# haowenz/FEM

Hardware: AMD Instinct MI355X
Metric: mapped Mreads/s (100 bp, e=3) at 1/2/4/8 MI355X + achieved HBM GB/s vs roofline (higher is better)
Workload: dtype u32/u64 integer + 32-bit Myers bit-vectors

## Files before the change

### fem_amd/csrc/fem_hip.hip

```cpp
#include "../../include/fem_hip.h"

#include <hip/hip_runtime.h>
#include <rccl/rccl.h>
#include <sched.h>
#if defined(__x86_64__)
#include <immintrin.h>
#endif

#include <algorithm>
#include <cctype>
#include <cstdio>
#include <cstdlib>
#include <cstring>
#include <condition_variable>
#include <functional>
#include <memory>
#include <atomic>
#include <chrono>
#include <mutex>
#include <string>
#include <thread>
#include <utility>
#include <vector>

// ... 199 lines not shown
  int n_cu = 256;
  std::string err;
  Buf<uint32_t> d_lookup;
  uint64_t n_lookup = 0;
  Buf<uint64_t> d_occ;
  uint64_t n_occ = 0;
  int32_t k = 0, step = 0;
  uint64_t fast_occ_key = ~0ull;
  int fast_occ_blocks = 0;
  Buf<uint32_t> d_summary;
  Buf<uint32_t> d_occ32, d_goff, d_blkseq;
  uint32_t list_shift = 0;
  bool no_strided = false;
  bool select_chars = false;
  bool verify_chars = false;
  Buf<uint32_t> d_freq11;
  uint32_t n_banks = 1, bank_first[5] = {0, 0, 0, 0, 0};
  Buf<uint32_t> d_bank_lo;
  uint64_t bank_limit = 0;
  uint32_t bank_seqs = 0;
  int select_occ_blocks = 0, join_occ_blocks = 0;
  uint64_t select_occ_key = ~0ull, join_occ_key = ~0ull;
  Buf<uint8_t> d_planes;
  Buf<uint8_t> d_ref_raw;
  uint64_t ref_bytes = 0;
  Buf<uint64_t> d_seq_off;
  Buf<uint32_t> d_seq_len;
  uint32_t n_seq = 0;
  std::vector<uint64_t> seq_off;
  std::vector<uint32_t> seq_len;
  Slot slot[kSlots];
// ... 167 lines not shown
    return at;
  };
  l.sf = take(2u * 64u * 4u);
  l.X = take(64u * 4u);
  l.A = take(3u * (femk::dense_flag_cap((int)R) + 1u) * 4u);
  l.B = take(2u * femk::kReadBlock * 8u);
  l.F = take(femk::join_bitmap_words((int)R, padded) * 4u);
  if (banked) l.gq = take(2u * 64u * 8u);
  l.wave_bytes = o;
  l.picked = 0;
  return l;
}

typedef void (*SeedKernel)(femk::SeedParams);
template <size_t... I>
SeedKernel select_kernel_of(int R, bool banked, bool packed, std::index_sequence<I...>) {
  static const SeedKernel k[2][2][femk::kMaxR] = {
      {{femk::seed_select_kernel<(int)I + 1, false, false>...}, {femk::seed_select_kernel<(int)I + 1, true, false>...}},
      {{femk::seed_select_kernel<(int)I + 1, false, true>...}, {femk::seed_select_kernel<(int)I + 1, true, true>...}}};
  return k[packed][banked][std::min(std::max(R, 1), femk::kMaxR) - 1];
}
template <size_t... I>
SeedKernel fast_kernel_of(int R, bool hash, std::index_sequence<I...>) {
  static const SeedKernel k[2][femk::kMaxR] = {{femk::seed_fast_kernel<(int)I + 1, false>...}, {femk::seed_fast_kernel<(int)I + 1, true>...}};
  return k[hash][std::min(std::max(R, 1), femk::kMaxR) - 1];
}
SeedKernel select_kernel(int R, bool banked, bool packed) { return select_kernel_of(R, banked, packed, std::make_index_sequence<femk::kMaxR>{}); }
SeedKernel fast_kernel(int R, bool hash) { return fast_kernel_of(R, hash, std::make_index_sequence<femk::kMaxR>{}); }
SeedKernel join_kernel(int R, int which) {
  static const SeedKernel k[3][femk::kMaxR] = {
      {femk::seed_join_kernel_r1, femk::seed_join_kernel_r2, femk::seed_join_kernel_r3, femk::seed_join_kernel_r4, femk::seed_join_kernel_r5,
       femk::seed_join_kernel_r6, femk::seed_join_kernel_r7, femk::seed_join_kernel_r8, femk::seed_join_kernel_r9, femk::seed_join_kernel_r10},
      {femk::seed_join_banked_kernel_r1, femk::seed_join_banked_kernel_r2, femk::seed_join_banked_kernel_r3, femk::seed_join_banked_kernel_r4,
       femk::seed_join_banked_kernel_r5, femk::seed_join_banked_kernel_r6, femk::seed_join_banked_kernel_r7, femk::seed_join_banked_kernel_r8,
       femk::seed_join_banked_kernel_r9, femk::seed_join_banked_kernel_r10},
      {femk::seed_join_kernel_padded_r1, femk::seed_join_kernel_padded_r2, femk::seed_join_kernel_padded_r3, femk::seed_join_kernel_padded_r4,
       femk::seed_join_kernel_padded_r5, femk::seed_join_kernel_padded_r6, femk::seed_join_kernel_padded_r7, femk::seed_join_kernel_padded_r8,
       femk::seed_join_kernel_padded_r9, femk::seed_join_kernel_padded_r10}};
  return k[which][std::min(std::max(R, 1), femk::kMaxR) - 1];
}

int blocks_per_cu(const void *kernel, int block, uint32_t lds) {
  int nb = 0;
  return hipOccupancyMaxActiveBlocksPerMultiprocessor(&nb, kernel, block, lds) == hipSuccess ? nb : 0;
}
uint32_t kernel_regs(int R, bool join, int which = 0, bool packed = false) {
  static std::atomic<uint32_t> cache[3][3][femk::kMaxR + 1] = {};
  std::atomic<uint32_t> &slot = cache[which][join ? 1 : packed ? 2 : 0][std::min(std::max(R, 1), femk::kMaxR)];
  uint32_t c = slot.load(std::memory_order_relaxed);
  if (c) return c;
  hipFuncAttributes a{};
  const void *f = join ? (const void *)join_kernel(R, which) : (const void *)select_kernel(R, which == 1, packed);
  c = hipFuncGetAttributes(&a, f) == hipSuccess && a.numRegs > 0 ? (uint32_t)a.numRegs : 128u;
  slot.store(c, std::memory_order_relaxed);
  return c;
}
void launch_select(int R, bool banked, dim3 grid, dim3 block, uint32_t lds, hipStream_t st, const femk::SeedParams &sp) {
  hipLaunchKernelGGL(select_kernel(R, banked, sp.packed != nullptr), grid, block, lds, st, sp);
}
void launch_join(int R, int which, dim3 grid, dim3 block, uint32_t lds, hipStream_t st, const femk::SeedParams &sp) {
  hipLaunchKernelGGL(join_kernel(R, which), grid, block, lds, st, sp);
}
void launch_fast(int R, bool hash, dim3 grid, dim3 block, uint32_t lds, hipStream_t st, const femk::SeedParams &sp) {
  hipLaunchKernelGGL(fast_kernel(R, hash), grid, block, lds, st, sp);
}

struct Span {
  fem_dev *h;
  Slot &s;
  hipStream_t st;
  TimedLaunch t;
  bool on;
  Span(fem_dev *h_, Slot &s_, int id, hipStream_t st_) : h(h_), s(s_), st(st_), t{id, nullptr, nullptr, false}, on(h_->timing && h_->timeline) {
// ... 153 lines not shown
}

int ensure_chars(fem_dev *h, Slot &s);

int launch_batch(fem_dev *h, Slot &s) {
  const fem_params &p = s.params;
  uint32_t *d_ctr = (uint32_t *)s.d_ctl.get();
  unsigned long long *d_arena_ctr = (unsigned long long *)(s.d_ctl + 4 * sizeof(uint32_t));
  unsigned long long *d_stats = (unsigned long long *)(s.d_ctl + 4 * sizeof(uint32_t) + 2 * sizeof(uint64_t));
  int parts = 1;
  uint32_t part_begin[kMaxParts + 1] = {0, 0, 0, 0, 0};
  const bool copied_in_parts = s.parts > 1;
  {
    const int R_ = p.e + 1 + p.a;
    const bool dense_overlap = !h->force_generic && p.k == femk::kK && p.step == femk::kStep && R_ >= 1 && R_ <= femk::kMaxR && h->d_occ32 &&
                               h->d_freq11 && !h->no_overlap;
    if (dense_overlap && !h->no_parts && s.n_reads >= 2 * kPartMinReads && (copied_in_parts || device_idle(h))) {
      parts = copied_in_parts ? s.parts : (int)std::min<uint64_t>((uint64_t)h->max_parts, s.n_reads / kPartMinReads);
      for (int q = 0; q <= parts; ++q)
        part_begin[q] = copied_in_parts ? s.part_begin[q] : q == parts ? (uint32_t)s.n_reads : (uint32_t)((s.n_reads * q / parts) & ~63ull);
    }
    s.parts = 1;
  }
  if (parts > 1) {
    if (h->have_select_done) HIP_TRY(h, hipStreamWaitEvent(h->side_stream, h->ev_select_done, 0));
    HIP_TRY(h, hipMemsetAsync(s.d_ctl, 0, kCtlAlloc, h->side_stream));
  } else {
    HIP_TRY(h, hipMemsetAsync(s.d_ctl, 0, kCtlAlloc, s.stream));
  }

  const int R_all = p.e + 1 + p.a;
  const bool dense_kernels = !h->force_generic && p.k == femk::kK && p.step == femk::kStep && R_all >= 1 && R_all <= femk::kMaxR && h->d_occ32 && h->d_freq11;
  if (s.n_reads && (!dense_kernels || h->verify_chars)) {
    int rc = ensure_chars(h, s);
    if (rc) return rc;
  }
  femk::SeedParams sp{};
  s.select_packed = false;
  if (s.sent_packed && !h->select_chars && dense_kernels) {
    sp.packed = s.packed(), sp.exc_bits = s.d_exc_bits, sp.bpr = s.packed_bpr, sp.len = s.max_len;
    s.select_packed = s.n_reads != 0;
  }
  sp.bases = s.bases();
  sp.read_off = s.d_off;
  sp.n_reads = (uint32_t)s.n_reads;
  sp.read_begin = 0;
  sp.lookup = h->d_lookup;
// ... 18 lines not shown
  const bool use_fast = !h->force_generic && p.k == femk::kK && p.step == femk::kStep && R >= 1 && R <= femk::kMaxR;

  auto shape = [&](const femk::SeedLayout &lay, uint32_t *wpb_out, uint32_t *lds_out, uint32_t *grid_out) {
    uint32_t wpb = std::min<uint32_t>(4u, std::max<uint32_t>(1u, (64u * 1024u) / lay.wave_bytes));
    uint32_t lds_bytes = wpb * lay.wave_bytes;
    uint32_t waves_per_cu = std::min<uint32_t>(32u, (160u * 1024u / lds_bytes) * wpb);
    uint64_t blocks_wanted = (s.n_reads + wpb - 1) / wpb;
    uint64_t blocks_resident = (uint64_t)h->n_cu * std::max<uint32_t>(1u, waves_per_cu / wpb);
    *wpb_out = wpb, *lds_out = lds_bytes;
    *grid_out = (uint32_t)std::max<uint64_t>(1, std::min<uint64_t>(blocks_wanted, blocks_resident * 4));
  };
  if (sp.lay.wave_bytes > 64u * 1024u) return fail(h, FEM_ERR_UNSUPPORTED, "read too long for the device path");

  if (s.n_reads) {
    int rc;
    const bool split_dense = use_fast && h->d_occ32 && h->d_freq11;
    const bool overlap = split_dense && !h->no_overlap;
    if (!overlap && h->have_kernels_done) HIP_TRY(h, hipStreamWaitEvent(s.stream, h->ev_kernels_done, 0));
    femk::VerifyParams vp{};
    vp.bases = s.bases(), vp.read_off = s.d_off;
    vp.planes = h->d_planes, vp.seq_off = h->d_seq_off;
    vp.cand = s.d_cand, vp.cand_meta = s.d_meta;
    vp.ctr = d_ctr, vp.cand_cap = s.cand_cap, vp.e = p.e;
    vp.ed = s.d_ed, vp.end = s.d_end;
    vp.n_map = s.d_nmap, vp.stats = d_stats;
    HIP_TRY(h, hipMemsetAsync(s.d_nmap, 0, (size_t)s.n_reads * sizeof(uint32_t), s.stream));
    const bool verify_packed = s.sent_packed && !h->verify_chars;
    if (verify_packed) vp.packed = s.packed(), vp.exc_bits = s.d_exc_bits, vp.bpr = s.packed_bpr, vp.len = s.max_len;
    void (*const verify)(femk::VerifyParams) = verify_packed ? femk::verify_kernel_packed : femk::verify_kernel;
    int &v_per_cu = verify_packed ? h->verify_packed_blocks_per_cu : h->verify_blocks_per_cu;
    if (v_per_cu == 0) {
      const int nb = blocks_per_cu((const void *)verify, 256, 0);
      v_per_cu = nb > 0 ? nb : 4;
    }
    const uint32_t vgrid = (uint32_t)h->n_cu * (uint32_t)v_per_cu;
    if (split_dense) {
      const uint32_t max_len = std::max<uint32_t>(s.max_len, (uint32_t)p.k);
      const bool banked = h->n_banks > 1;
      const size_t want_sel = (size_t)s.n_reads * 6u * (size_t)R * h->n_banks;
      HIP_TRY(h, s.d_sel.ensure(want_sel));
      HIP_TRY(h, s.d_sel_hdr.ensure((size_t)s.n_reads));
      femk::SeedParams fp = sp;
      fp.occ32 = h->d_occ32, fp.list_shift = h->list_shift, fp.goff = h->d_goff, fp.blkseq = h->d_blkseq;
      fp.freq11 = h->d_freq11, fp.sel = s.d_sel, fp.sel_hdr = s.d_sel_hdr;
      fp.n_banks = h->n_banks, fp.bank_lo = h->d_bank_lo, fp.n_buckets = (uint32_t)(h->n_lookup - 1);
      fp.blk_stride = (femk::kDenseRemap >> femk::kDenseBlkShift) + 1u;
      for (uint32_t b = 0; b <= femk::kDenseMaxBanks; ++b) fp.bank_first[b] = h->bank_first[b];
      uint32_t select_lds = 0, select_threads = 256;
      fp.lay = make_layout_select(p, max_len, fp.packed != nullptr);
      if (fp.lay.wave_bytes > 64u * 1024u) return fail(h, FEM_ERR_UNSUPPORTED, "read too long for the device path");
      const femk::SeedLayout lay_select = fp.lay;
      femk::SeedLayout lay_join = make_layout_join(p, banked, !banked && h->list_shift != 0);
      const uint32_t wpb_s = std::min<uint32_t>(4u, std::max<uint32_t>(1u, (64u * 1024u) / lay_select.wave_bytes));
      const uint32_t wpb_j = std::min<uint32_t>(4u, std::max<uint32_t>(1u, (60u * 1024u) / lay_join.wave_bytes));
      lay_join.picked = wpb_j * lay_join.wave_bytes;
      const uint32_t lds_j = wpb_j * lay_join.wave_bytes + 64u * 8u;
      const int which = banked ? 1 : h->list_shift ? 2 : 0;
      uint64_t per_cu_s, per_cu_j;
      {
        const uint32_t lds_bytes = wpb_s * lay_select.wave_bytes;
        const uint64_t key = ((uint64_t)(fp.packed != nullptr) << 49) | ((uint64_t)banked << 48) | ((uint64_t)R << 40) | lds_bytes;
        if (h->select_occ_key != key)
          h->select_occ_key = key, h->select_occ_blocks = blocks_per_cu((const void *)select_kernel(R, banked, fp.packed != nullptr), (int)(64u * wpb_s), lds_bytes);
        per_cu_s = h->select_occ_blocks > 0 ? (uint64_t)h->select_occ_blocks : std::max<uint64_t>(1, 160u * 1024u / lds_bytes);
        if (overlap) per_cu_s = 1;
        select_lds = lds_bytes, select_threads = 64u * wpb_s;
      }
      {
        const uint64_t key = ((uint64_t)which << 48) | ((uint64_t)R << 40) | lds_j;
        if (h->join_occ_key != key) h->join_occ_key = key, h->join_occ_blocks = blocks_per_cu((const void *)join_kernel(R, which), (int)(64u * wpb_j), lds_j);
        per_cu_j = h->join_occ_blocks > 0 ? (uint64_t)h->join_occ_blocks : std::max<uint64_t>(1, 160u * 1024u / lds_j);
        if (overlap) {
          const uint32_t vj = (kernel_regs(R, true, which) + 7u) & ~7u, vs = (kernel_regs(R, false, banked ? 1 : 0, fp.packed != nullptr) + 7u) & ~7u;
          const uint32_t wj = 64u * wpb_j / 256u ? 64u * wpb_j / 256u : 1u, ws = select_threads / 256u ? select_threads / 256u : 1u;
          const uint32_t lj = (lds_j + 511u) & ~511u, ls = (select_lds + 511u) & ~511u;
          while (per_cu_j > 1 && (per_cu_j * wj * vj + ws * vs > 512u || per_cu_j * lj + ls > 160u * 1024u || per_cu_j * wj + ws > 8u)) --per_cu_j;
        }
      }
      if (parts > 1 && !copied_in_parts) {
        HIP_TRY(h, hipEventRecord(s.ev_zeroed, s.stream));
        HIP_TRY(h, hipStreamWaitEvent(h->side_stream, s.ev_zeroed, 0));
      }
      for (int q = 0; q < parts; ++q) {
        const uint32_t r_lo = parts > 1 ? part_begin[q] : 0u, r_hi = parts > 1 ? part_begin[q + 1] : (uint32_t)s.n_reads;
        const uint64_t blocks_of_reads = ((uint64_t)(r_hi - r_lo) + femk::kReadBlock - 1) / femk::kReadBlock;
        fp.read_begin = r_lo, fp.n_reads = r_hi;
        hipStream_t st_sel = parts > 1 ? h->side_stream : s.stream;
        {
          fp.lay = lay_select;
          if (parts > 1) {
            if (copied_in_parts) HIP_TRY(h, hipStreamWaitEvent(st_sel, s.ev_part[q], 0));
          } else if (overlap && h->have_select_done) {
            HIP_TRY(h, hipStreamWaitEvent(s.stream, h->ev_select_done, 0));
          }
          const uint32_t grid = (uint32_t)std::max<uint64_t>(1, std::min<uint64_t>((blocks_of_reads + wpb_s - 1) / wpb_s, (uint64_t)h->n_cu * per_cu_s));
          fp.work_cursor = (uint32_t *)(s.d_ctl + kCtlWorkCursor + (size_t)q * kCtlPartStride);
          rc = timed_launch(h, s, 8, st_sel, q == 0, [&] { launch_select(R, banked, dim3(grid), dim3(64u * wpb_s), select_lds, st_sel, fp); });
          if (rc) return rc;
          if (parts > 1) {
            HIP_TRY(h, hipEventRecord(s.ev_sel[q], st_sel));
            HIP_TRY(h, hipStreamWaitEvent(s.stream, s.ev_sel[q], 0));
          }
          if (overlap && q + 1 == parts) {
            HIP_TRY(h, hipEventRecord(h->ev_select_done, st_sel));
            h->have_select_done = true;
          }
          if (overlap && q == 0 && h->have_kernels_done) HIP_TRY(h, hipStreamWaitEvent(s.stream, h->ev_kernels_done, 0));
        }
        {
          fp.lay = lay_join;
          const uint32_t grid = (uint32_t)std::max<uint64_t>(1, std::min<uint64_t>((blocks_of_reads + wpb_j - 1) / wpb_j, (uint64_t)h->n_cu * per_cu_j));
          fp.work_cursor = (uint32_t *)(s.d_ctl + kCtlWorkCursor2 + (size_t)q * kCtlPartStride);
// ... 75 lines not shown
  h->d_summary.release();
  const uint64_t n_buckets = h->n_lookup - 1;
  if (h->n_occ >= n_buckets || h->n_occ >= 0x80000000ull || (n_buckets >> 3) >= (1ull << 22)) return FEM_OK;
  const uint64_t words = n_buckets / femk::kSummaryBuckets + 2;
  HIP_TRY(h, h->d_summary.ensure(words));
  HIP_TRY(h, hipMemset(h->d_summary, 0, words * sizeof(uint32_t)));
  hipLaunchKernelGGL(femk::bucket_summary_kernel, dim3((uint32_t)h->n_cu * 8u), dim3(256), 0, 0, h->d_lookup, n_buckets, h->d_summary);
  HIP_TRY(h, hipGetLastError());
  HIP_TRY(h, hipDeviceSynchronize());
  return FEM_OK;
}

constexpr double kDenseMinAvgBucket = 4.0;
int refresh_dense(fem_dev *h) {
  auto drop = [&]() {
    h->d_occ32.release(), h->d_goff.release(), h->d_blkseq.release(), h->d_freq11.release(), h->d_bank_lo.release();
    h->n_banks = 1, h->list_shift = 0;
  };
  drop();
  if (!h->d_occ || !h->d_ref_raw || h->no_dense || h->k != femk::kK || h->step != femk::kStep || h->n_occ == 0) return FEM_OK;
  const uint64_t n_buckets = h->n_lookup - 1;
  if (!h->force_dense && (double)h->n_occ < kDenseMinAvgBucket * (double)n_buckets) return FEM_OK;
  const uint64_t limit = h->bank_limit ? std::min<uint64_t>(h->bank_limit, femk::kDenseLimit) : femk::kDenseLimit;
  const uint32_t seq_limit = h->bank_seqs ? std::min<uint32_t>(h->bank_seqs, femk::kDenseMaxSeq) : femk::kDenseMaxSeq;
  std::vector<uint32_t> goff(h->n_seq + 1);
  uint32_t n_banks = 1, bank_first[5] = {0, 0, 0, 0, 0};
  uint64_t cap = limit;
  {
    uint64_t total_c = femk::kDenseGap, longest = 0;
    for (uint32_t i = 0; i < h->n_seq; ++i) total_c += (uint64_t)h->seq_len[i] + femk::kDenseGap, longest = std::max<uint64_t>(longest, h->seq_len[i]);
    const uint64_t want = (total_c + limit - 1) / limit;
// ... 31 lines not shown
  if (n_banks == 1 && !h->no_strided && strided_pays) {
    const size_t words = ((size_t)n_buckets + femk::kDensePadBuckets) << femk::kDenseListShift;
    bool ok = h->d_occ32.ensure(words) == hipSuccess;
    if (ok) {
      hipLaunchKernelGGL(femk::dense_pad_kernel, dim3((uint32_t)h->n_cu * 16u), dim3(256), 0, 0, (uint4 *)h->d_occ32.get(), (uint64_t)(words / 4));
      ok = hipGetLastError() == hipSuccess;
    }
    if (ok) {
      list_shift = femk::kDenseListShift;
    } else {
      h->d_occ32.release();
      (void)hipGetLastError();
    }
  }
  if (h->d_goff.ensure(goff.size()) != hipSuccess || h->d_blkseq.ensure(blkseq.size()) != hipSuccess ||
      (!list_shift && h->d_occ32.ensure(h->n_occ + 256) != hipSuccess) || h->d_freq11.ensure((size_t)femk::kX11 * 4u) != hipSuccess ||
      (n_banks > 1 && h->d_bank_lo.ensure((size_t)(n_banks - 1) * n_buckets) != hipSuccess) || d_bad.ensure(1) != hipSuccess)
    return decline();
  if (hipMemset(d_bad, 0, sizeof(uint32_t)) != hipSuccess ||
      hipMemcpy(h->d_goff, goff.data(), goff.size() * sizeof(uint32_t), hipMemcpyHostToDevice) != hipSuccess ||
      hipMemcpy(h->d_blkseq, blkseq.data(), blkseq.size() * sizeof(uint32_t), hipMemcpyHostToDevice) != hipSuccess) {
    (void)decline();
    return fail(h, FEM_ERR_HIP, "dense tables: copy to the device failed");
  }
  femk::BankFirst bf{};
  bf.n = n_banks;
  for (uint32_t b = 0; b <= femk::kDenseMaxBanks; ++b) bf.first[b] = bank_first[b];
  if (list_shift)
    hipLaunchKernelGGL(femk::dense_occ32_strided_kernel, dim3((uint32_t)h->n_cu * 8u), dim3(256), 0, 0, h->d_occ, h->d_lookup, (uint32_t)n_buckets, h->d_goff,
                       h->n_seq, h->d_occ32, d_bad);
  else
    hipLaunchKernelGGL(femk::dense_occ32_kernel, dim3((uint32_t)h->n_cu * 8u), dim3(256), 0, 0, h->d_occ, h->n_occ, h->d_goff, h->n_seq, bf,
                       h->d_occ32, d_bad);
  uint32_t bad = 0;
  if (hipGetLastError() != hipSuccess || hipMemcpy(&bad, d_bad, sizeof bad, hipMemcpyDeviceToHost) != hipSuccess) {
    (void)decline();
    return fail(h, FEM_ERR_HIP, "dense tables: building the 32-bit occurrence table failed");
  }
  if (bad) return decline();
  d_bad.release();
  for (uint32_t b = 1; b < n_banks; ++b)
    hipLaunchKernelGGL(femk::bank_split_kernel, dim3((uint32_t)h->n_cu * 8u), dim3(256), 0, 0, h->d_occ, h->d_lookup, (uint32_t)n_buckets, bank_first[b],
                       h->d_bank_lo + (size_t)(b - 1) * n_buckets);
  h->n_banks = n_banks, h->list_shift = list_shift;
  for (uint32_t b = 0; b <= femk::kDenseMaxBanks; ++b) h->bank_first[b] = bank_first[b];
  hipLaunchKernelGGL(femk::freq11_kernel, dim3((uint32_t)h->n_cu * 8u), dim3(256), 0, 0, h->d_lookup, h->d_freq11);
  HIP_TRY(h, hipGetLastError());
  HIP_TRY(h, hipDeviceSynchronize());
  return FEM_OK;
}

struct CommSet {
  std::vector<int> devs;
  std::vector<ncclComm_t> comms;
  std::vector<Buf<uint64_t>> bufs;
};
std::mutex g_comm_mu;
CommSet *g_comm = nullptr;
void destroy_comm_set() {
  if (!g_comm) return;
  for (size_t i = 0; i < g_comm->devs.size(); ++i) {
// ... 47 lines not shown
int enqueue_packed(fem_dev *h, Slot &s, uint64_t n, uint32_t len, uint64_t n_exc) {
  const uint32_t bpr = fempack::bytes_per_read(len);
  const uint64_t code_bytes = fempack::code_bytes(n, len), n_bases = n * (uint64_t)len;
  const uint64_t total = code_bytes + n_exc * 5u;
  int rc;
  HIP_TRY(h, s.d_packed_alloc.ensure(kPackedFrontPad + (size_t)total + 64));
  HIP_TRY(h, s.d_bases_alloc.ensure(kFrontPad + (size_t)n_bases + 64));
  HIP_TRY(h, s.d_off.ensure((size_t)n + 1));
  HIP_TRY(h, s.d_exc_bits.ensure((size_t)n / 32 + 2));
  s.parts = 1;
  if (!h->no_parts && !h->no_overlap && n_exc == 0 && n >= 2 * kPartMinReads && device_idle(h))
    s.parts = (int)std::min<uint64_t>((uint64_t)h->max_parts, n / kPartMinReads);
  for (int q = 0; q <= s.parts; ++q) s.part_begin[q] = q == s.parts ? (uint32_t)n : (uint32_t)((n * q / s.parts) & ~63ull);
  HIP_TRY(h, hipMemsetAsync(s.d_exc_bits, 0, ((size_t)n / 32 + 1) * sizeof(uint32_t), s.stream));
  const bool at_commit = h->select_chars || n_exc * kExpandAllShare > n;
  const bool offs_at_commit = at_commit || !(h->d_occ32 && h->d_freq11);
  if (offs_at_commit)
    hipLaunchKernelGGL(femk::uniform_offsets_kernel, dim3((uint32_t)std::min<uint64_t>((n + 256) / 256, (uint64_t)h->n_cu * 8u)), dim3(256), 0,
                       s.stream, s.d_off, n, len);
  if ((rc = h2d_begin(h, s))) return rc;
  for (int q = 0; q < s.parts; ++q) {
    const uint64_t r0 = s.part_begin[q], r1 = s.part_begin[q + 1];
    const uint64_t b0 = r0 * bpr, b1 = q + 1 == s.parts ? total : r1 * bpr;
    Span span(h, s, 20, s.stream);
    if (b1 > b0) HIP_TRY(h, hipMemcpyAsync(s.packed() + b0, s.h_bases + b0, b1 - b0, hipMemcpyHostToDevice, s.stream));
    if (q + 1 == s.parts && (rc = h2d_end(h, s))) return rc;
    if (at_commit && r1 > r0) {
      const uint32_t grid = (uint32_t)std::min<uint64_t>(((r1 - r0) * bpr + 255) / 256, (uint64_t)h->n_cu * 16u);
      hipLaunchKernelGGL(femk::unpack_reads_kernel, dim3(grid), dim3(256), 0, s.stream, (const uint8_t *)s.packed() + b0, r1 - r0, len, bpr,
                         s.bases() + r0 * len);
    }
// ... 89 lines not shown
  }
  if (testing_switch("FEM_TESTING")) {
    h->no_overlap = testing_switch("FEM_NO_OVERLAP");
    h->no_parts = testing_switch("FEM_NO_PARTS");
    if (const char *mp = getenv("FEM_PARTS")) h->max_parts = std::min(kMaxParts, std::max(1, atoi(mp)));
    h->timeline = testing_switch("FEM_TIMELINE");
    if (h->timeline && h->ev_epoch.create() == hipSuccess && hipEventRecord(h->ev_epoch, h->side_stream) == hipSuccess)
      h->timing = true, h->have_epoch = true;
    h->force_generic = testing_switch("FEM_FORCE_GENERIC");
    h->force_hash = testing_switch("FEM_FORCE_HASH");
    h->force_dense = testing_switch("FEM_FORCE_DENSE");
    h->no_dense = testing_switch("FEM_NO_DENSE");
    h->no_strided = testing_switch("FEM_NO_STRIDED");
    h->verify_chars = testing_switch("FEM_VERIFY_CHARS");
    h->select_chars = testing_switch("FEM_SELECT_CHARS");
    h->tiny_buffers = testing_switch("FEM_TEST_TINY_BUFFERS");
    if (const char *bl = getenv("FEM_TEST_BANK_BASES")) h->bank_limit = strtoull(bl, nullptr, 10);
    if (const char *bs = getenv("FEM_TEST_BANK_SEQS")) h->bank_seqs = (uint32_t)strtoul(bs, nullptr, 10);
  }
  *out = h;
  return FEM_OK;
}

int fem_dev_close(fem_dev *h) {
  if (!h) return FEM_ERR_INVALID;
  {
    std::lock_guard<std::mutex> lock(g_comm_mu);
    if (g_comm && std::find(g_comm->devs.begin(), g_comm->devs.end(), h->device) != g_comm->devs.end()) destroy_comm_set();
  }
  (void)hipSetDevice(h->device);
// ... 572 lines not shown
  if (n_reads == 0 || n_reads > 0x7FFFFFF0ull || n_records > 0xFFFFFFF0ull || max_len == 0 || max_len > kMaxReadLen)
    return fail(h, FEM_ERR_INVALID, "batch shape out of range");
  Slot &s = h->slot[slot];
  if (s.mapped && !s.synced) return fail(h, FEM_ERR_STATE, "a batch is in flight in this slot");
  HIP_TRY(h, hipSetDevice(h->device));
  const uint64_t n_was = s.n_reads;
  s.n_reads = n_reads;
  rc = ensure_outputs(h, s);
  s.n_reads = n_was;
  if (rc) return rc;
  const uint64_t n_bases = n_reads * (uint64_t)max_len;
  HIP_TRY(h, s.d_packed_alloc.ensure(kPackedFrontPad + (size_t)fempack::code_bytes(n_reads, max_len) + 64));
  HIP_TRY(h, s.d_bases_alloc.ensure(kFrontPad + (size_t)n_bases + 64));
  HIP_TRY(h, s.d_off.ensure((size_t)n_reads + 1));
  HIP_TRY(h, s.d_exc_bits.ensure((size_t)n_reads / 32 + 2));
  if (h->d_occ32 && h->d_freq11 && p->k == 12 && p->step == 3) {
    const size_t R = (size_t)(p->e + 1 + p->a);
    HIP_TRY(h, s.d_sel.ensure((size_t)n_reads * 6u * R * h->n_banks));
    HIP_TRY(h, s.d_sel_hdr.ensure((size_t)n_reads));
  }
  if (!s.tail) s.tail.reset(new (std::nothrow) femt::Tail());
  if (!s.tail) return fail(h, FEM_ERR_NOMEM, "out of host memory");
  std::string err;
  if ((rc = s.tail->reserve((uint32_t)n_reads, (uint32_t)n_records, max_len, p->e, h->tiny_buffers, &err))) return fail(h, rc, err);
  if (!s.text_stream) HIP_TRY(h, s.text_stream.create(hipStreamNonBlocking));
  HIP_TRY(h, hipMemsetAsync(s.d_sel_hdr ? (void *)s.d_sel_hdr.get() : (void *)s.d_off.get(), 0, 8, s.text_stream));
  HIP_TRY(h, hipStreamSynchronize(s.text_stream));
  HIP_TRY(h, hipMemsetAsync(s.d_off, 0, 8, h->side_stream));
  HIP_TRY(h, hipStreamSynchronize(h->side_stream));
  const size_t probe = 1u << 20;
  if (s.h_bases && s.h_bases.size() >= probe && s.d_bases_alloc.size() >= kFrontPad + probe)
// ... 383 lines not shown

int fem_dev_map_batch_submit(fem_dev *h, int slot, const fem_params *p, const fem_read_batch *reads) {
  int rc = fem_dev_stage_reads(h, slot, reads);
  if (rc) return rc;
  return fem_dev_map_staged(h, slot, p);
}

int fem_dev_map_batch_wait(fem_dev *h, int slot, fem_batch_result *out) { return fem_dev_fetch(h, slot, out); }

int fem_dev_index_info(const fem_dev *h, char *buf, uint64_t cap) {
  if (!h || !buf || cap == 0) return FEM_ERR_INVALID;
  const uint64_t n_buckets = h->n_lookup ? h->n_lookup - 1 : 0;
  std::string s;
  if (!h->d_lookup) {
    s = "no index";
  } else if (h->d_occ32 && h->d_freq11) {
    s = "dense: 32-bit occurrence table, ";
    s += h->list_shift ? "strided with pads (" + std::to_string(((n_buckets + femk::kDensePadBuckets) << h->list_shift) * 4 >> 20) + " MiB)"
                       : "compact (" + std::to_string(h->n_occ * 4 >> 20) + " MiB)";
    s += ", " + std::to_string(h->n_banks) + (h->n_banks == 1 ? " bank" : " banks") + ", freq11 64 MiB";
  } else if (h->d_summary) {
    s = "sparse: bucket summaries";
  } else {
    s = "64-bit occurrence table only";
  }
  s += "; " + std::to_string(h->n_occ) + " entries in " + std::to_string(n_buckets) + " buckets";
  snprintf(buf, (size_t)cap, "%s", s.c_str());
  return FEM_OK;
}

const char *fem_dev_seed_kernel(const fem_dev *h, const fem_params *p) {
  if (!h || !params_ok(p)) return "";
  const int R = p->e + 1 + p->a;
  const bool use_fast = !h->force_generic && p->k == femk::kK && p->step == femk::kStep && R >= 1 && R <= femk::kMaxR;
  if (!use_fast) return "seed_filter_kernel";
  if (h->d_occ32 && h->d_freq11) return h->n_banks > 1 ? "seed_join_banked_kernel" : "seed_join_kernel";
  return (h->force_hash || (double)h->n_occ > (double)h->n_lookup) ? "seed_fast_kernel<hash>" : "seed_fast_kernel<lean>";
}

int fem_dev_set_timing(fem_dev *h, int on) {
  if (!h) return FEM_ERR_INVALID;
  h->timing = on != 0;
  if (h->timing && h->event_pool.idle.size() < 64) {
    HIP_TRY(h, hipSetDevice(h->device));
    HIP_TRY(h, h->event_pool.fill(64));
  }
  return FEM_OK;
}

int fem_dev_reset_timing(fem_dev *h) {
  if (!h) return FEM_ERR_INVALID;
// ... 190 lines not shown
```

### fem_amd/csrc/fem_kernels.hip.h

```cpp
#pragma once
#include <hip/hip_runtime.h>
#include <stdint.h>
#include "fem_planes.hip.h"

namespace femk {

constexpr int kWave = 64;
constexpr uint32_t kFlagCandOverflow = 1u;
constexpr uint32_t kFlagArenaOverflow = 2u;
constexpr uint32_t kFlagTooLarge = 4u;
constexpr uint32_t kInvalidMeta = 0xFFFFFFFFu;
constexpr int kMaxR = 10;
constexpr uint32_t kMeta16 = 0x80000000u;
constexpr uint32_t kSlotChunk = 256u;
constexpr uint32_t kFlagQueueOverflow = 8u;
constexpr uint32_t kQueueChunk = 32u;
constexpr uint32_t kInvalidRead = 0xFFFFFFFFu;

struct SeedLayout {
  uint32_t pkw, nkw;
  uint32_t sf;
  uint32_t dp_rows;
  uint32_t dp_bits;
  uint32_t picked;
// ... 24 lines not shown
  uint64_t *cand;
  uint32_t *cand_meta;
  uint32_t cand_cap;
  uint32_t *cand_begin;
  uint32_t *cand_count;
  uint32_t *ctr;
  uint32_t n_seq;
  uint32_t *slow_queue;
  uint32_t slow_cap;
  const uint32_t *work_queue;
  const uint32_t *summary;
  const uint32_t *occ32;
  uint32_t list_shift;
  const uint32_t *goff;
  const uint32_t *blkseq;
  const uint32_t *freq11;
  uint2 *sel;
  uint2 *sel_hdr;
  uint32_t n_banks;
  uint32_t bank_first[5];
  const uint32_t *bank_lo;
  uint32_t n_buckets;
  uint32_t blk_stride;
  unsigned long long *stats;
  uint64_t *arena;
  unsigned long long arena_cap;
  unsigned long long *arena_ctr;
  SeedLayout lay;
  const uint8_t *packed;
  const uint32_t *exc_bits;
  uint32_t bpr, len;
// ... 1228 lines not shown
```

### fem_amd/csrc/fem_seed_select.hip.h

```cpp
#pragma once
#include <type_traits>

#include "fem_seed_fast.hip.h"

namespace femk {

constexpr uint32_t kDenseMaxBanks = 4;
constexpr uint32_t kDenseNear = 1024u;
constexpr uint32_t kDenseRemap = 0xF0000000u;
constexpr uint32_t kSelKeepAll = 1u << 15;
constexpr uint32_t kSelOk = 0u, kSelNone = 1u, kSelSlow = 2u;
constexpr uint32_t kSelMaxCols = 128u;
constexpr uint32_t kSelMaxList = 128u;
constexpr uint32_t kX11 = 1u << 22;

__device__ __forceinline__ uint32_t wave_min_u32(uint32_t x) {
  constexpr uint32_t kFill = 0xFFFFFFFFu;
  x = dpp_min_step<0x111, 0xF>(x, kFill), x = dpp_min_step<0x112, 0xF>(x, kFill), x = dpp_min_step<0x114, 0xF>(x, kFill);
  x = dpp_min_step<0x118, 0xF>(x, kFill), x = dpp_min_step<0x142, 0xA>(x, kFill), x = dpp_min_step<0x143, 0xC>(x, kFill);
  return (uint32_t)__builtin_amdgcn_readlane((int)x, 63);
}
__device__ __forceinline__ uint32_t wave_max_u32(uint32_t x) {
  return (uint32_t)__builtin_amdgcn_readlane((int)wave_scan_max(x), 63);
}
// ... 23 lines not shown
  asm("" : "+v"(twice));
  return __builtin_amdgcn_alignbit(w[0], w[1], 0u - twice);
}
__device__ __forceinline__ uint32_t div3_small(uint32_t x) { return __umul24(x, 21846u) >> 16; }
__device__ __forceinline__ uint32_t div6_small(uint32_t x) { return __umul24(x, 10923u) >> 16; }
__device__ __forceinline__ uint32_t times3(uint32_t x) {
  uint32_t r;
  asm("v_lshl_add_u32 %0, %1, 1, %1" : "=v"(r) : "v"(x));
  return r;
}
__device__ __forceinline__ uint32_t rc_hash(uint32_t hf, uint32_t nm) {
  const uint32_t r = __brev((~hf) & ~nm & kHashMask) >> (32 - 2 * kK);
  return ((r & 0x55555555u) << 1) | ((r >> 1) & 0x55555555u);
}

template <int R, int W>
__device__ __forceinline__ void select_dp(const uint16_t *F, uint32_t ncols, uint32_t maxcols, uint32_t inf, uint32_t (&take)[R][W],
                                          uint32_t &m_last, uint32_t &iters) {
  uint32_t M[R];
#pragma unroll
  for (int r = 0; r < R; ++r) {
    M[r] = inf;
#pragma unroll
    for (int w = 0; w < W; ++w) take[r][w] = 0;
  }
  for (uint32_t c = 0; c < maxcols; ++c) {
    uint32_t f[R];
#pragma unroll
    for (int r = 0; r < R; ++r) f[r] = F[3u * c + 12u * (uint32_t)r];
    const bool in = c < ncols;
// ... 32 lines not shown
};
__device__ __forceinline__ PackedArgs packed_args() {
  typedef const __attribute__((address_space(4))) SeedParams *ArgPtr;
  ArgPtr a = (ArgPtr)__builtin_amdgcn_kernarg_segment_ptr();
  asm volatile("" : "+s"(a));
  return {a->packed, a->bases, a->exc_bits, a->bpr, a->len};
}

#ifndef FEM_SELECT_WAVES
#define FEM_SELECT_WAVES 6
#endif
#ifndef FEM_SELECT_UNROLL
#define FEM_SELECT_UNROLL 2
#endif

template <int R, bool BANKED = false, bool PACKED = false>
__global__ void __launch_bounds__(256) __attribute__((amdgpu_waves_per_eu(FEM_SELECT_WAVES, 8))) seed_select_kernel(SeedParams p) {
  extern __shared__ __attribute__((aligned(16))) uint8_t smem[];
  const uint32_t ln = lane_id();
  const uint32_t wave_in_block = (uint32_t)__builtin_amdgcn_readfirstlane((int)(threadIdx.x >> 6));
  uint8_t *wbase = smem + (size_t)wave_in_block * p.lay.wave_bytes;
  uint64_t *boff = (uint64_t *)(wbase + p.lay.rb);
  uint32_t *fw = (uint32_t *)(wbase + p.lay.strm);
  uint32_t *nw = fw + p.lay.strm_words;
  uint16_t *fq = (uint16_t *)(wbase + p.lay.fq);
  uint32_t *r_base = (uint32_t *)(wbase + p.lay.rinfo), *r_len = r_base + kReadBlock, *r_flag = r_len + kReadBlock,
           *r_pre = r_flag + kReadBlock;
  constexpr uint32_t kOk0 = 1u, kOk1 = 2u, kShape = 4u, kSlow = 8u;
  const uint32_t sstride = p.lay.gstride, nb = p.lay.nb;
  const uint32_t inf = p.inf32;
  SlotChunk qchunk;
// ... 123 lines not shown
              n_f += isn & (uint32_t)(at >= (uint32_t)kK);
              n_r += isn & (uint32_t)(L - 1u - at >= (uint32_t)kK);
            }
          }
          for (int d = 32; d >= 1; d >>= 1) n_f += __shfl_xor(n_f, d), n_r += __shfl_xor(n_r, d);
          if (ln == 0) {
            uint32_t fl = r_flag[i];
            if (n_f > (uint32_t)p.e) fl &= ~kOk0;
            if (n_r > (uint32_t)p.e) fl &= ~kOk1;
            r_flag[i] = fl;
          }
        }
        wave_sync_lds();
      }
      const uint32_t SP = wave_max_u32(my_S);
      if (SP != 0) {
        const uint32_t SPp = (SP + 1u) >> 1;
        const uint32_t magic = 0xFFFFFFFFu / SPp + 1u;
        const uint32_t total = cnt * SPp;
        constexpr int U = FEM_SELECT_UNROLL;
        constexpr uint32_t kActBit = 1u << 25, kTwoBit = 1u << 24;
        for (uint32_t w0 = 0; w0 < total; w0 += (uint32_t)(U * kWave)) {
          uint32_t d0[U], d1[U], where[U];
#pragma unroll
          for (int u = 0; u < U; ++u) {
            const uint32_t w = w0 + (uint32_t)(u * kWave) + ln;
            const uint32_t i = __umulhi(w, magic);
            const uint32_t j = (w - __umul24(i, SPp)) << 1;
            const uint32_t i_c = i < cnt ? i : 0u;
            const uint32_t fl = r_flag[i_c];
            const uint32_t S = r_len[i_c] - (uint32_t)(kK - 1);
            const bool act = w < total && (fl & kShape) && !(fl & kSlow) && j < S;
            const bool two = act && j + 1u < S;
            const uint32_t win = stream_window(fw, act ? r_base[i_c] + j : 0u);
            const uint32_t hf0 = win >> 8;
            const uint32_t at0 = ((hf0 & (kX11 - 1u)) << 2) | (hf0 >> 22), at1 = (win >> 6) & kHashMask;
            d0[u] = p.freq11[act ? at0 : 0u];
            d1[u] = p.freq11[two ? at1 : 0u];
            where[u] = i_c | (j << 4) | (S << 14) | (two ? kTwoBit : 0u) | (act ? kActBit : 0u);
          }
#pragma unroll
          for (int u = 0; u < U; ++u) {
            if (where[u] & kActBit) {
              const uint32_t i = where[u] & 15u, j = (where[u] >> 4) & 1023u, S = (where[u] >> 14) & 1023u;
              const bool two = (where[u] & kTwoBit) != 0u;
              uint32_t x = (d0[u] & 0x0000FFFFu) | (d1[u] & 0xFFFF0000u);
              if (!two) x &= 0x0000FFFFu;
              uint32_t ffwd = x & 0x00FF00FFu, frev = (x >> 8) & 0x00FF00FFu;
              const uint32_t is255 = ((x & 0x7F7F7F7Fu) + 0x01010101u) & x & 0x80808080u;
              if (has_n || is255 != 0u) {
                uint32_t f2[2] = {0u, 0u}, r2[2] = {0u, 0u};
#pragma unroll
                for (int q = 0; q < 2; ++q) {
// ... 161 lines not shown
```

Baseline: 400.5.

## Add freq10 table so each window lookup serves three k-mer positions

```diff
diff --git a/fem_amd/csrc/fem_hip.hip b/fem_amd/csrc/fem_hip.hip
--- a/fem_amd/csrc/fem_hip.hip
+++ b/fem_amd/csrc/fem_hip.hip
@@ -237,7 +237,8 @@
   bool no_strided = false;
   bool select_chars = false;
   bool verify_chars = false;
-  Buf<uint32_t> d_freq11;
+  bool select_freq11 = false;
+  Buf<uint32_t> d_freq;
   uint32_t n_banks = 1, bank_first[5] = {0, 0, 0, 0, 0};
   Buf<uint32_t> d_bank_lo;
   uint64_t bank_limit = 0;
@@ -435,18 +436,22 @@
 
 typedef void (*SeedKernel)(femk::SeedParams);
 template <size_t... I>
-SeedKernel select_kernel_of(int R, bool banked, bool packed, std::index_sequence<I...>) {
-  static const SeedKernel k[2][2][femk::kMaxR] = {
-      {{femk::seed_select_kernel<(int)I + 1, false, false>...}, {femk::seed_select_kernel<(int)I + 1, true, false>...}},
-      {{femk::seed_select_kernel<(int)I + 1, false, true>...}, {femk::seed_select_kernel<(int)I + 1, true, true>...}}};
-  return k[packed][banked][std::min(std::max(R, 1), femk::kMaxR) - 1];
+SeedKernel select_kernel_of(int R, bool banked, bool packed, bool pairs, std::index_sequence<I...>) {
+  static const SeedKernel k[2][2][2][femk::kMaxR] = {
+      {{{femk::seed_select_kernel<(int)I + 1, false, false, false>...}, {femk::seed_select_kernel<(int)I + 1, true, false, false>...}},
+       {{femk::seed_select_kernel<(int)I + 1, false, true, false>...}, {femk::seed_select_kernel<(int)I + 1, true, true, false>...}}},
+      {{{femk::seed_select_kernel<(int)I + 1, false, false, true>...}, {femk::seed_select_kernel<(int)I + 1, true, false, true>...}},
+       {{femk::seed_select_kernel<(int)I + 1, false, true, true>...}, {femk::seed_select_kernel<(int)I + 1, true, true, true>...}}}};
+  return k[pairs][packed][banked][std::min(std::max(R, 1), femk::kMaxR) - 1];
 }
 template <size_t... I>
 SeedKernel fast_kernel_of(int R, bool hash, std::index_sequence<I...>) {
   static const SeedKernel k[2][femk::kMaxR] = {{femk::seed_fast_kernel<(int)I + 1, false>...}, {femk::seed_fast_kernel<(int)I + 1, true>...}};
   return k[hash][std::min(std::max(R, 1), femk::kMaxR) - 1];
 }
-SeedKernel select_kernel(int R, bool banked, bool packed) { return select_kernel_of(R, banked, packed, std::make_index_sequence<femk::kMaxR>{}); }
+SeedKernel select_kernel(int R, bool banked, bool packed, bool pairs) {
+  return select_kernel_of(R, banked, packed, pairs, std::make_index_sequence<femk::kMaxR>{});
+}
 SeedKernel fast_kernel(int R, bool hash) { return fast_kernel_of(R, hash, std::make_index_sequence<femk::kMaxR>{}); }
 SeedKernel join_kernel(int R, int which) {
   static const SeedKernel k[3][femk::kMaxR] = {
@@ -465,19 +470,19 @@
   int nb = 0;
   return hipOccupancyMaxActiveBlocksPerMultiprocessor(&nb, kernel, block, lds) == hipSuccess ? nb : 0;
 }
-uint32_t kernel_regs(int R, bool join, int which = 0, bool packed = false) {
-  static std::atomic<uint32_t> cache[3][3][femk::kMaxR + 1] = {};
-  std::atomic<uint32_t> &slot = cache[which][join ? 1 : packed ? 2 : 0][std::min(std::max(R, 1), femk::kMaxR)];
+uint32_t kernel_regs(int R, bool join, int which = 0, bool packed = false, bool pairs = false) {
+  static std::atomic<uint32_t> cache[3][5][femk::kMaxR + 1] = {};
+  std::atomic<uint32_t> &slot = cache[which][join ? 1 : (packed ? 2 : 0) + (pairs ? 3 : 0)][std::min(std::max(R, 1), femk::kMaxR)];
   uint32_t c = slot.load(std::memory_order_relaxed);
   if (c) return c;
   hipFuncAttributes a{};
-  const void *f = join ? (const void *)join_kernel(R, which) : (const void *)select_kernel(R, which == 1, packed);
+  const void *f = join ? (const void *)join_kernel(R, which) : (const void *)select_kernel(R, which == 1, packed, pairs);
   c = hipFuncGetAttributes(&a, f) == hipSuccess && a.numRegs > 0 ? (uint32_t)a.numRegs : 128u;
   slot.store(c, std::memory_order_relaxed);
   return c;
 }
-void launch_select(int R, bool banked, dim3 grid, dim3 block, uint32_t lds, hipStream_t st, const femk::SeedParams &sp) {
-  hipLaunchKernelGGL(select_kernel(R, banked, sp.packed != nullptr), grid, block, lds, st, sp);
+void launch_select(int R, bool banked, bool pairs, dim3 grid, dim3 block, uint32_t lds, hipStream_t st, const femk::SeedParams &sp) {
+  hipLaunchKernelGGL(select_kernel(R, banked, sp.packed != nullptr, pairs), grid, block, lds, st, sp);
 }
 void launch_join(int R, int which, dim3 grid, dim3 block, uint32_t lds, hipStream_t st, const femk::SeedParams &sp) {
   hipLaunchKernelGGL(join_kernel(R, which), grid, block, lds, st, sp);
@@ -661,7 +666,7 @@
   {
     const int R_ = p.e + 1 + p.a;
     const bool dense_overlap = !h->force_generic && p.k == femk::kK && p.step == femk::kStep && R_ >= 1 && R_ <= femk::kMaxR && h->d_occ32 &&
-                               h->d_freq11 && !h->no_overlap;
+                               h->d_freq && !h->no_overlap;
     if (dense_overlap && !h->no_parts && s.n_reads >= 2 * kPartMinReads && (copied_in_parts || device_idle(h))) {
       parts = copied_in_parts ? s.parts : (int)std::min<uint64_t>((uint64_t)h->max_parts, s.n_reads / kPartMinReads);
       for (int q = 0; q <= parts; ++q)
@@ -677,7 +682,7 @@
   }
 
   const int R_all = p.e + 1 + p.a;
-  const bool dense_kernels = !h->force_generic && p.k == femk::kK && p.step == femk::kStep && R_all >= 1 && R_all <= femk::kMaxR && h->d_occ32 && h->d_freq11;
+  const bool dense_kernels = !h->force_generic && p.k == femk::kK && p.step == femk::kStep && R_all >= 1 && R_all <= femk::kMaxR && h->d_occ32 && h->d_freq;
   if (s.n_reads && (!dense_kernels || h->verify_chars)) {
     int rc = ensure_chars(h, s);
     if (rc) return rc;
@@ -726,7 +731,7 @@
 
   if (s.n_reads) {
     int rc;
-    const bool split_dense = use_fast && h->d_occ32 && h->d_freq11;
+    const bool split_dense = use_fast && h->d_occ32 && h->d_freq;
     const bool overlap = split_dense && !h->no_overlap;
     if (!overlap && h->have_kernels_done) HIP_TRY(h, hipStreamWaitEvent(s.stream, h->ev_kernels_done, 0));
     femk::VerifyParams vp{};
@@ -754,7 +759,7 @@
       HIP_TRY(h, s.d_sel_hdr.ensure((size_t)s.n_reads));
       femk::SeedParams fp = sp;
       fp.occ32 = h->d_occ32, fp.list_shift = h->list_shift, fp.goff = h->d_goff, fp.blkseq = h->d_blkseq;
-      fp.freq11 = h->d_freq11, fp.sel = s.d_sel, fp.sel_hdr = s.d_sel_hdr;
+      fp.freq = h->d_freq, fp.sel = s.d_sel, fp.sel_hdr = s.d_sel_hdr;
       fp.n_banks = h->n_banks, fp.bank_lo = h->d_bank_lo, fp.n_buckets = (uint32_t)(h->n_lookup - 1);
       fp.blk_stride = (femk::kDenseRemap >> femk::kDenseBlkShift) + 1u;
       for (uint32_t b = 0; b <= femk::kDenseMaxBanks; ++b) fp.bank_first[b] = h->bank_first[b];
@@ -773,7 +778,7 @@
         const uint32_t lds_bytes = wpb_s * lay_select.wave_bytes;
         const uint64_t key = ((uint64_t)(fp.packed != nullptr) << 49) | ((uint64_t)banked << 48) | ((uint64_t)R << 40) | lds_bytes;
         if (h->select_occ_key != key)
-          h->select_occ_key = key, h->select_occ_blocks = blocks_per_cu((const void *)select_kernel(R, banked, fp.packed != nullptr), (int)(64u * wpb_s), lds_bytes);
+          h->select_occ_key = key, h->select_occ_blocks = blocks_per_cu((const void *)select_kernel(R, banked, fp.packed != nullptr, h->select_freq11), (int)(64u * wpb_s), lds_bytes);
         per_cu_s = h->select_occ_blocks > 0 ? (uint64_t)h->select_occ_blocks : std::max<uint64_t>(1, 160u * 1024u / lds_bytes);
         if (overlap) per_cu_s = 1;
         select_lds = lds_bytes, select_threads = 64u * wpb_s;
@@ -783,7 +788,7 @@
         if (h->join_occ_key != key) h->join_occ_key = key, h->join_occ_blocks = blocks_per_cu((const void *)join_kernel(R, which), (int)(64u * wpb_j), lds_j);
         per_cu_j = h->join_occ_blocks > 0 ? (uint64_t)h->join_occ_blocks : std::max<uint64_t>(1, 160u * 1024u / lds_j);
         if (overlap) {
-          const uint32_t vj = (kernel_regs(R, true, which) + 7u) & ~7u, vs = (kernel_regs(R, false, banked ? 1 : 0, fp.packed != nullptr) + 7u) & ~7u;
+          const uint32_t vj = (kernel_regs(R, true, which) + 7u) & ~7u, vs = (kernel_regs(R, false, banked ? 1 : 0, fp.packed != nullptr, h->select_freq11) + 7u) & ~7u;
           const uint32_t wj = 64u * wpb_j / 256u ? 64u * wpb_j / 256u : 1u, ws = select_threads / 256u ? select_threads / 256u : 1u;
           const uint32_t lj = (lds_j + 511u) & ~511u, ls = (select_lds + 511u) & ~511u;
           while (per_cu_j > 1 && (per_cu_j * wj * vj + ws * vs > 512u || per_cu_j * lj + ls > 160u * 1024u || per_cu_j * wj + ws > 8u)) --per_cu_j;
@@ -807,7 +812,7 @@
           }
           const uint32_t grid = (uint32_t)std::max<uint64_t>(1, std::min<uint64_t>((blocks_of_reads + wpb_s - 1) / wpb_s, (uint64_t)h->n_cu * per_cu_s));
           fp.work_cursor = (uint32_t *)(s.d_ctl + kCtlWorkCursor + (size_t)q * kCtlPartStride);
-          rc = timed_launch(h, s, 8, st_sel, q == 0, [&] { launch_select(R, banked, dim3(grid), dim3(64u * wpb_s), select_lds, st_sel, fp); });
+          rc = timed_launch(h, s, 8, st_sel, q == 0, [&] { launch_select(R, banked, h->select_freq11, dim3(grid), dim3(64u * wpb_s), select_lds, st_sel, fp); });
           if (rc) return rc;
           if (parts > 1) {
             HIP_TRY(h, hipEventRecord(s.ev_sel[q], st_sel));
@@ -913,7 +918,7 @@
 constexpr double kDenseMinAvgBucket = 4.0;
 int refresh_dense(fem_dev *h) {
   auto drop = [&]() {
-    h->d_occ32.release(), h->d_goff.release(), h->d_blkseq.release(), h->d_freq11.release(), h->d_bank_lo.release();
+    h->d_occ32.release(), h->d_goff.release(), h->d_blkseq.release(), h->d_freq.release(), h->d_bank_lo.release();
     h->n_banks = 1, h->list_shift = 0;
   };
   drop();
@@ -975,7 +980,7 @@
     }
   }
   if (h->d_goff.ensure(goff.size()) != hipSuccess || h->d_blkseq.ensure(blkseq.size()) != hipSuccess ||
-      (!list_shift && h->d_occ32.ensure(h->n_occ + 256) != hipSuccess) || h->d_freq11.ensure((size_t)femk::kX11 * 4u) != hipSuccess ||
+      (!list_shift && h->d_occ32.ensure(h->n_occ + 256) != hipSuccess) || h->d_freq.ensure(h->select_freq11 ? (size_t)femk::kX11 * 4u : (size_t)femk::kY10 * 32u) != hipSuccess ||
       (n_banks > 1 && h->d_bank_lo.ensure((size_t)(n_banks - 1) * n_buckets) != hipSuccess) || d_bad.ensure(1) != hipSuccess)
     return decline();
   if (hipMemset(d_bad, 0, sizeof(uint32_t)) != hipSuccess ||
@@ -1005,7 +1010,10 @@
                        h->d_bank_lo + (size_t)(b - 1) * n_buckets);
   h->n_banks = n_banks, h->list_shift = list_shift;
   for (uint32_t b = 0; b <= femk::kDenseMaxBanks; ++b) h->bank_first[b] = bank_first[b];
-  hipLaunchKernelGGL(femk::freq11_kernel, dim3((uint32_t)h->n_cu * 8u), dim3(256), 0, 0, h->d_lookup, h->d_freq11);
+  if (h->select_freq11)
+    hipLaunchKernelGGL(femk::freq11_kernel, dim3((uint32_t)h->n_cu * 8u), dim3(256), 0, 0, h->d_lookup, h->d_freq);
+  else
+    hipLaunchKernelGGL(femk::freq10_kernel, dim3((uint32_t)h->n_cu * 8u), dim3(256), 0, 0, h->d_lookup, (uint16_t *)h->d_freq.get());
   HIP_TRY(h, hipGetLastError());
   HIP_TRY(h, hipDeviceSynchronize());
   return FEM_OK;
@@ -1083,7 +1091,7 @@
   for (int q = 0; q <= s.parts; ++q) s.part_begin[q] = q == s.parts ? (uint32_t)n : (uint32_t)((n * q / s.parts) & ~63ull);
   HIP_TRY(h, hipMemsetAsync(s.d_exc_bits, 0, ((size_t)n / 32 + 1) * sizeof(uint32_t), s.stream));
   const bool at_commit = h->select_chars || n_exc * kExpandAllShare > n;
-  const bool offs_at_commit = at_commit || !(h->d_occ32 && h->d_freq11);
+  const bool offs_at_commit = at_commit || !(h->d_occ32 && h->d_freq);
   if (offs_at_commit)
     hipLaunchKernelGGL(femk::uniform_offsets_kernel, dim3((uint32_t)std::min<uint64_t>((n + 256) / 256, (uint64_t)h->n_cu * 8u)), dim3(256), 0,
                        s.stream, s.d_off, n, len);
@@ -1203,6 +1211,7 @@
     h->no_strided = testing_switch("FEM_NO_STRIDED");
     h->verify_chars = testing_switch("FEM_VERIFY_CHARS");
     h->select_chars = testing_switch("FEM_SELECT_CHARS");
+    h->select_freq11 = testing_switch("FEM_SELECT_FREQ11");
     h->tiny_buffers = testing_switch("FEM_TEST_TINY_BUFFERS");
     if (const char *bl = getenv("FEM_TEST_BANK_BASES")) h->bank_limit = strtoull(bl, nullptr, 10);
     if (const char *bs = getenv("FEM_TEST_BANK_SEQS")) h->bank_seqs = (uint32_t)strtoul(bs, nullptr, 10);
@@ -1805,7 +1814,7 @@
   HIP_TRY(h, s.d_bases_alloc.ensure(kFrontPad + (size_t)n_bases + 64));
   HIP_TRY(h, s.d_off.ensure((size_t)n_reads + 1));
   HIP_TRY(h, s.d_exc_bits.ensure((size_t)n_reads / 32 + 2));
-  if (h->d_occ32 && h->d_freq11 && p->k == 12 && p->step == 3) {
+  if (h->d_occ32 && h->d_freq && p->k == 12 && p->step == 3) {
     const size_t R = (size_t)(p->e + 1 + p->a);
     HIP_TRY(h, s.d_sel.ensure((size_t)n_reads * 6u * R * h->n_banks));
     HIP_TRY(h, s.d_sel_hdr.ensure((size_t)n_reads));
@@ -2219,11 +2228,11 @@
   std::string s;
   if (!h->d_lookup) {
     s = "no index";
-  } else if (h->d_occ32 && h->d_freq11) {
+  } else if (h->d_occ32 && h->d_freq) {
     s = "dense: 32-bit occurrence table, ";
     s += h->list_shift ? "strided with pads (" + std::to_string(((n_buckets + femk::kDensePadBuckets) << h->list_shift) * 4 >> 20) + " MiB)"
                        : "compact (" + std::to_string(h->n_occ * 4 >> 20) + " MiB)";
-    s += ", " + std::to_string(h->n_banks) + (h->n_banks == 1 ? " bank" : " banks") + ", freq11 64 MiB";
+    s += ", " + std::to_string(h->n_banks) + (h->n_banks == 1 ? " bank" : " banks") + (h->select_freq11 ? ", freq11 64 MiB" : ", freq10 128 MiB");
   } else if (h->d_summary) {
     s = "sparse: bucket summaries";
   } else {
@@ -2239,7 +2248,7 @@
   const int R = p->e + 1 + p->a;
   const bool use_fast = !h->force_generic && p->k == femk::kK && p->step == femk::kStep && R >= 1 && R <= femk::kMaxR;
   if (!use_fast) return "seed_filter_kernel";
-  if (h->d_occ32 && h->d_freq11) return h->n_banks > 1 ? "seed_join_banked_kernel" : "seed_join_kernel";
+  if (h->d_occ32 && h->d_freq) return h->n_banks > 1 ? "seed_join_banked_kernel" : "seed_join_kernel";
   return (h->force_hash || (double)h->n_occ > (double)h->n_lookup) ? "seed_fast_kernel<hash>" : "seed_fast_kernel<lean>";
 }
 
diff --git a/fem_amd/csrc/fem_kernels.hip.h b/fem_amd/csrc/fem_kernels.hip.h
--- a/fem_amd/csrc/fem_kernels.hip.h
+++ b/fem_amd/csrc/fem_kernels.hip.h
@@ -62,7 +62,7 @@
   uint32_t list_shift;
   const uint32_t *goff;
   const uint32_t *blkseq;
-  const uint32_t *freq11;
+  const uint32_t *freq;
   uint2 *sel;
   uint2 *sel_hdr;
   uint32_t n_banks;
diff --git a/fem_amd/csrc/fem_seed_select.hip.h b/fem_amd/csrc/fem_seed_select.hip.h
--- a/fem_amd/csrc/fem_seed_select.hip.h
+++ b/fem_amd/csrc/fem_seed_select.hip.h
@@ -61,6 +61,21 @@
   return ((r & 0x55555555u) << 1) | ((r >> 1) & 0x55555555u);
 }
 
+constexpr uint32_t kY10 = 1u << 20;
+constexpr uint32_t kF10B = 32u, kF10C = 64u;
+__global__ void freq10_kernel(const uint32_t *lookup, uint16_t *freq10) {
+  const uint32_t stride = gridDim.x * blockDim.x;
+  for (uint32_t t = blockIdx.x * blockDim.x + threadIdx.x; t < kY10 * 64u; t += stride) {
+    const uint32_t Y = t >> 6, blk = (t >> 4) & 3u, c = t & 15u;
+    auto f = [&](uint32_t h) -> uint32_t {
+      const uint32_t d = lookup[h + 1u] - lookup[h];
+      return d < 255u ? d : 255u;
+    };
+    const uint32_t h = blk == 0u ? (c << 20) | Y : blk == 1u ? ((c >> 2) << 22) | (Y << 2) | (c & 3u) : (Y << 4) | c;
+    freq10[t] = blk < 3u ? (uint16_t)(f(h) | (f(rc_hash(h, 0u)) << 8)) : (uint16_t)0;
+  }
+}
+
 template <int R, int W>
 __device__ __forceinline__ void select_dp(const uint16_t *F, uint32_t ncols, uint32_t maxcols, uint32_t inf, uint32_t (&take)[R][W],
                                           uint32_t &m_last, uint32_t &iters) {
@@ -123,7 +138,7 @@
 #define FEM_SELECT_UNROLL 2
 #endif
 
-template <int R, bool BANKED = false, bool PACKED = false>
+template <int R, bool BANKED = false, bool PACKED = false, bool PAIRS = false>
 __global__ void __launch_bounds__(256) __attribute__((amdgpu_waves_per_eu(FEM_SELECT_WAVES, 8))) seed_select_kernel(SeedParams p) {
   extern __shared__ __attribute__((aligned(16))) uint8_t smem[];
   const uint32_t ln = lane_id();
@@ -277,6 +292,68 @@
         wave_sync_lds();
       }
       const uint32_t SP = wave_max_u32(my_S);
+      if constexpr (!PAIRS) {
+        if (SP != 0) {
+          const uint32_t SPt = div3_small(SP + 2u);
+          const uint32_t magic = 0xFFFFFFFFu / SPt + 1u;
+          const uint32_t total = cnt * SPt;
+          const uint8_t *table = (const uint8_t *)p.freq;
+          constexpr int U = FEM_SELECT_UNROLL;
+          constexpr uint32_t kActBit = 1u << 25, kTwoBit = 1u << 24, kThreeBit = 1u << 26;
+          for (uint32_t w0 = 0; w0 < total; w0 += (uint32_t)(U * kWave)) {
+            uint32_t d0[U], d1[U], d2[U], where[U];
+#pragma unroll
+            for (int u = 0; u < U; ++u) {
+              const uint32_t w = w0 + (uint32_t)(u * kWave) + ln;
+              const uint32_t i = __umulhi(w, magic);
+              const uint32_t j = times3(w - __umul24(i, SPt));
+              const uint32_t i_c = i < cnt ? i : 0u;
+              const uint32_t fl = r_flag[i_c];
+              const uint32_t S = r_len[i_c] - (uint32_t)(kK - 1);
+              const bool act = w < total && (fl & kShape) && !(fl & kSlow) && j < S;
+              const uint32_t win = stream_window(fw, act ? r_base[i_c] + j : 0u);
+              const uint32_t line = (win >> 1) & ((kY10 - 1u) << 7);
+              d0[u] = *(const uint16_t *)(table + (line | ((win >> 27) & 0x1Eu)));
+              d1[u] = *(const uint16_t *)(table + (line | kF10B | ((win >> 25) & 0x18u) | ((win >> 5) & 0x06u)));
+              d2[u] = *(const uint16_t *)(table + (line | kF10C | ((win >> 3) & 0x1Eu)));
+              where[u] = i_c | (j << 4) | (S << 14) | (act && j + 1u < S ? kTwoBit : 0u) | (act && j + 2u < S ? kThreeBit : 0u) |
+                         (act ? kActBit : 0u);
+            }
+#pragma unroll
+            for (int u = 0; u < U; ++u) {
+              if (where[u] & kActBit) {
+                const uint32_t i = where[u] & 15u, j = (where[u] >> 4) & 1023u, S = (where[u] >> 14) & 1023u;
+                const bool two = (where[u] & kTwoBit) != 0u, three = (where[u] & kThreeBit) != 0u;
+                const uint32_t x = d0[u] | (two ? d1[u] << 16 : 0u), y = three ? d2[u] : 0u;
+                uint32_t f3[3] = {x & 255u, (x >> 16) & 255u, y & 255u}, r3[3] = {(x >> 8) & 255u, x >> 24, y >> 8};
+                const uint32_t is255 = (((x & 0x7F7F7F7Fu) + 0x01010101u) & x & 0x80808080u) | (((y & 0x7F7Fu) + 0x0101u) & y & 0x8080u);
+                if (has_n || is255 != 0u) {
+#pragma unroll
+                  for (int q = 0; q < 3; ++q) {
+                    if ((q == 1 && !two) || (q == 2 && !three)) continue;
+                    uint32_t f_fwd = f3[q], f_rev = r3[q];
+                    const uint32_t pos = r_base[i] + j + (uint32_t)q;
+                    const uint32_t hf = stream_window(fw, pos) >> 8;
+                    const uint32_t nm = has_n ? stream_window(nw, pos) >> 8 : 0u;
+                    if (f_fwd == 255u) f_fwd = p.lookup[hf + 1u] - p.lookup[hf];
+                    if (nm != 0u || f_rev == 255u) {
+                      const uint32_t hr = rc_hash(hf, nm);
+                      f_rev = p.lookup[hr + 1u] - p.lookup[hr];
+                    }
+                    if (f_fwd >= 0xFFFFu || f_rev >= 0xFFFFu) atomicOr(&r_flag[i], kSlow);
+                    f3[q] = f_fwd < 0xFFFFu ? f_fwd : 0xFFFFu, r3[q] = f_rev < 0xFFFFu ? f_rev : 0xFFFFu;
+                  }
+                }
+                uint16_t *row_f = fq + __umul24(i, 2u * sstride), *row_r = row_f + sstride;
+                const uint32_t jr = S - 1u - j;
+                row_f[j] = (uint16_t)f3[0], row_r[jr] = (uint16_t)r3[0];
+                if (two) row_f[j + 1u] = (uint16_t)f3[1], row_r[jr - 1u] = (uint16_t)r3[1];
+                if (three) row_f[j + 2u] = (uint16_t)f3[2], row_r[jr - 2u] = (uint16_t)r3[2];
+              }
+            }
+          }
+        }
+      } else
       if (SP != 0) {
         const uint32_t SPp = (SP + 1u) >> 1;
         const uint32_t magic = 0xFFFFFFFFu / SPp + 1u;
@@ -298,8 +375,8 @@
             const uint32_t win = stream_window(fw, act ? r_base[i_c] + j : 0u);
             const uint32_t hf0 = win >> 8;
             const uint32_t at0 = ((hf0 & (kX11 - 1u)) << 2) | (hf0 >> 22), at1 = (win >> 6) & kHashMask;
-            d0[u] = p.freq11[act ? at0 : 0u];
-            d1[u] = p.freq11[two ? at1 : 0u];
+            d0[u] = p.freq[act ? at0 : 0u];
+            d1[u] = p.freq[two ? at1 : 0u];
             where[u] = i_c | (j << 4) | (S << 14) | (two ? kTwoBit : 0u) | (act ? kActBit : 0u);
           }
 #pragma unroll
```

After: 400.0. No clear change (-0.1%).
